# mjq11302010044/TPGSR

Hardware: AMD Instinct MI355X
Metric: training img/s (16x64->32x128, bs=48/GPU), TPGSR-TSRN full train step (higher is better)
Workload: dtype bf16x2; 1 GPU; C3: TPGSR-TSRN = TSRN_TL (STN+mask) + CRNN teacher/student text prior, stu_iter 1, full train step (teacher fwd, student fwd+bwd, distill loss, prior dropout, SR fwd+bwd, ImageLoss(gradient), clip 0.25, Adam); tpg=crnn, batch_per_gpu=48, global_batch=48, parallelism=dp1, launch=recorded plans, plain launches: main + weight-gradient + teacher streams

## Files before the change

### tpgsr_amd/csrc/gru_wgrad.hip

```cpp
#include "conv_xbf_common.h"
#include <mutex>
#include <stdlib.h>

#define GW_PITCH 832
#define GW_ROWS 32
#define GW_PLANE (GW_ROWS * GW_PITCH)
#define GW_HP 96
#define GW_GI 160
#define GW_GN 352

__device__ __forceinline__ bf16x8 gw_frag(const unsigned char* plane, int lane, int col0, int mb) {
  const int G = lane >> 4, q = lane & 15;
  const int mbase = mb * 16 + (G >> 1) * 8;
  const int c0 = col0 + (G & 1) * 16 + (q & 3) * 4;
  const unsigned char* p = plane + (mbase + (q >> 2)) * GW_PITCH + c0 * 2;
  s16x4 lo = __builtin_amdgcn_ds_read_tr16_b64_v4i16((lds_s16x4_ptr)(p));
  s16x4 hi = __builtin_amdgcn_ds_read_tr16_b64_v4i16((lds_s16x4_ptr)(p + 4 * GW_PITCH));
  typedef short s16x8 __attribute__((ext_vector_type(8)));
  s16x8 v = __builtin_shufflevector(lo, hi, 0, 1, 2, 3, 4, 5, 6, 7);
  return __builtin_bit_cast(bf16x8, v);
}

template <int LD, int T, int KB>
__global__ __launch_bounds__(384) void gru_wgrad_kernel(tpgsr_gru_wgrad_args w, int P, int MB) {
  extern __shared__ __attribute__((aligned(16))) unsigned char gsm[];
  const tpgsr_conv_args& a = w.c;
  const int tid = threadIdx.x;
  const int lane = tid & 63, wave = __builtin_amdgcn_readfirstlane(tid >> 6);
  const int z = blockIdx.x, Z = gridDim.x;
  const int mbeg = z * MB, mend = min(P, mbeg + MB);
  constexpr int QA = KB * 8;

  const bool doA = tid < 16 * QA;
  const int a_cq = doA ? tid % QA : 0, a_r0 = doA ? tid / QA : 0;
  const bool doH = tid < 256;
  const int h_cq = tid & 15, h_r0 = (tid >> 4) & 15;
  const bool doN = tid >= 128;
  const int n_cq = (tid - 128) & 15, n_r0 = ((tid - 128) >> 4) & 15;
  const int g_cq = tid % 48, g_r0 = tid / 48;

  const size_t in_floats = (size_t)a.N * a.H * a.W * a.in_ld;
  const __amdgpu_buffer_rsrc_t rs_in = make_rsrc(a.in, in_floats);
  const __amdgpu_buffer_rsrc_t rs_in2 = (LD & 16) ? make_rsrc(a.in_b, (size_t)a.N * a.W * a.in_b_ld)
                                                  : make_rsrc(a.in2 ? a.in2 : a.in, (size_t)a.N * a.H * a.W * a.in2_ld);
  const __amdgpu_buffer_rsrc_t rs_h = make_rsrc(w.h, (size_t)P * 64);
  const __amdgpu_buffer_rsrc_t rs_gi = make_rsrc(w.dgi, (size_t)P * 192);
  const __amdgpu_buffer_rsrc_t rs_gn = make_rsrc(w.dghn, (size_t)P * 64);
  float4 qs = make_float4(1.f, 1.f, 1.f, 1.f), qt = make_float4(0.f, 0.f, 0.f, 0.f);
  if ((LD & 1) && doA) {
    qs = *reinterpret_cast<const float4*>(a.in_scale + a_cq * 4);
    qt = *reinterpret_cast<const float4*>(a.in_shift + a_cq * 4);
  }
  const KPos kp = {0, 0, a_cq * 4};
  const int hd = h_cq >> 3;
  const int hstep = (w.axis == 0 ? 1 : a.W) * (hd == 0 ? -1 : 1);

  ARaw ra[2];
  float4 rh[2], rn[2], rg[4];
  float4 dbq = make_float4(0.f, 0.f, 0.f, 0.f), dbn = make_float4(0.f, 0.f, 0.f, 0.f);
  auto load_chunk = [&](const int mc) __attribute__((always_inline)) {
#pragma unroll
    for (int i = 0; i < 2; ++i) {
      if (doA) {
        const PixelPos p = decode_pixel(a, mc + a_r0 + 16 * i, mend);
        ra[i] = load_a_raw<LD>(a, rs_in, rs_in2, p, kp);
      }
      if (doH) {
        const int m = mc + h_r0 + 16 * i;
        const PixelPos p = decode_pixel(a, m, mend);
        const int pos = w.axis == 0 ? p.ow : p.oh, last = (w.axis == 0 ? a.W : a.H) - 1;
        const bool ok = p.valid && (hd == 0 ? pos > 0 : pos < last);
        rh[i] = buf_load4(rs_h, ok ? ((unsigned)(m + hstep) * 64u + (unsigned)(h_cq * 4)) * 4u : OOB_OFF);
      }
      if (doN) {
        const int m = mc + n_r0 + 16 * i;
        rn[i] = buf_load4(rs_gn, m < mend ? ((unsigned)m * 64u + (unsigned)(n_cq * 4)) * 4u : OOB_OFF);
      }
    }
#pragma unroll
    for (int i = 0; i < 4; ++i) {
      const int m = mc + g_r0 + 8 * i;
      rg[i] = buf_load4(rs_gi, m < mend ? ((unsigned)m * 192u + (unsigned)(g_cq * 4)) * 4u : OOB_OFF);
    }
  };
  auto put = [&](const float4& v, const int row, const int col) __attribute__((always_inline)) {
    uint2 hsp[T];
    split4<T>(v, hsp);
#pragma unroll
    for (int t = 0; t < T; ++t) *reinterpret_cast<uint2*>(gsm + t * GW_PLANE + row * GW_PITCH + col * 2) = hsp[t];
  };
  auto store_chunk = [&]() __attribute__((always_inline)) {
#pragma unroll
    for (int i = 0; i < 2; ++i) {
      if (doA) put(finish_a<LD>(a, ra[i], qs, qt), a_r0 + 16 * i, a_cq * 4);
      if (doH) put(rh[i], h_r0 + 16 * i, GW_HP + h_cq * 4);
      if (doN) {
        put(rn[i], n_r0 + 16 * i, GW_GN + n_cq * 4);
        dbn.x += rn[i].x; dbn.y += rn[i].y; dbn.z += rn[i].z; dbn.w += rn[i].w;
      }
    }
#pragma unroll
    for (int i = 0; i < 4; ++i) {
      put(rg[i], g_r0 + 8 * i, GW_GI + g_cq * 4);
      dbq.x += rg[i].x; dbq.y += rg[i].y; dbq.z += rg[i].z; dbq.w += rg[i].w;
    }
  };

  const int d = wave / 3, g = wave - 3 * d;
  floatx16 acc[KB], acch;
#pragma unroll
  for (int r = 0; r < 16; ++r) {
    acch[r] = 0.f;
#pragma unroll
    for (int kb = 0; kb < KB; ++kb) acc[kb][r] = 0.f;
  }

  if (mbeg < mend) {
    load_chunk(mbeg);
    store_chunk();
  }
  __syncthreads();
  for (int mc = mbeg; mc < mend; mc += GW_ROWS) {
    const bool more = mc + GW_ROWS < mend;
    if (more) load_chunk(mc + GW_ROWS);
#pragma unroll
    for (int mb = 0; mb < GW_ROWS / 16; ++mb) {
      bf16x8 by[T], byh[T], av[T];
#pragma unroll
      for (int t = 0; t < T; ++t) by[t] = gw_frag(gsm + t * GW_PLANE, lane, GW_GI + 32 * wave, mb);
      if (g == 2) {
#pragma unroll
        for (int t = 0; t < T; ++t) byh[t] = gw_frag(gsm + t * GW_PLANE, lane, GW_GN + 32 * d, mb);
      } else {
#pragma unroll
        for (int t = 0; t < T; ++t) byh[t] = by[t];
      }
#pragma unroll
      for (int kb = 0; kb < KB; ++kb) {
#pragma unroll
        for (int t = 0; t < T; ++t) av[t] = gw_frag(gsm + t * GW_PLANE, lane, 32 * kb, mb);
        acc[kb] = mfma_terms<T>(av, by, acc[kb]);
      }
#pragma unroll
      for (int t = 0; t < T; ++t) av[t] = gw_frag(gsm + t * GW_PLANE, lane, GW_HP + 32 * d, mb);
      acch = mfma_terms<T>(av, byh, acch);
    }
    __builtin_amdgcn_sched_barrier(0);
    __syncthreads();
    if (more) {
      store_chunk();
      __syncthreads();
    }
  }

  const int col = lane & 31;
#pragma unroll
  for (int kb = 0; kb < KB; ++kb) {
    float* dst = w.partC + ((size_t)z * a.Cin + 32 * kb) * 192 + 32 * wave + col;
#pragma unroll
    for (int r = 0; r < 16; ++r) dst[(size_t)((r & 3) + 8 * (r >> 2) + 4 * (lane >> 5)) * 192] = acc[kb][r];
  }
  {
    float* dst = w.partH + ((size_t)d * Z + z) * 32 * 96 + 32 * g + col;
#pragma unroll
    for (int r = 0; r < 16; ++r) dst[(size_t)((r & 3) + 8 * (r >> 2) + 4 * (lane >> 5)) * 96] = acch[r];
  }
  float* red = reinterpret_cast<float*>(gsm);
  float* redn = red + 8 * 192;
  *reinterpret_cast<float4*>(red + g_r0 * 192 + g_cq * 4) = dbq;
  if (doN) *reinterpret_cast<float4*>(redn + n_r0 * 64 + n_cq * 4) = dbn;
  __syncthreads();
  if (tid < 192) {
    float s = 0.f;
#pragma unroll
    for (int r = 0; r < 8; ++r) s += red[r * 192 + tid];
    w.dbC[(size_t)z * 192 + tid] = s;
    const int dd = tid / 96, c = tid - 96 * dd;
    if (c < 64) w.dbH[((size_t)dd * Z + z) * 96 + c] = s;
  } else if (tid < 256) {
    const int c = tid - 192;
    float s = 0.f;
#pragma unroll
    for (int r = 0; r < 16; ++r) s += redn[r * 64 + c];
    w.dbH[((size_t)(c >> 5) * Z + z) * 96 + 64 + (c & 31)] = s;
  }
}

static int g_gw_z = [] { const char* e = getenv("TPGSR_GRU_WGRAD_Z"); const int v = e ? atoi(e) : 128; return v > 0 ? v : 128; }();

extern "C" int tpgsr_gru_wgrad_splits(long long P) {
  long long z = g_gw_z;
  const long long maxz = (P + 63) / 64;
  if (z > maxz) z = maxz;
  if (z < 1) z = 1;
  const long long mb = ((P + z - 1) / z + GW_ROWS - 1) / GW_ROWS * GW_ROWS;
  return (int)((P + mb - 1) / mb);
}

extern "C" int tpgsr_gru_wgrad(const tpgsr_gru_wgrad_args* w, void* stream) {
  TPGSR_CHECK_ARG(w != nullptr, "tpgsr_gru_wgrad: null args");
  const tpgsr_conv_args* a = &w->c;
  TPGSR_CHECK_ARG(a->in && w->dgi && w->dghn && w->h && w->partC && w->partH && w->dbC && w->dbH, "tpgsr_gru_wgrad: null pointer");
  TPGSR_CHECK_ARG(a->N > 0 && a->H > 0 && a->W > 0 && (a->Cin == 64 || a->Cin == 96) && a->Cout == 192 && a->KH == 1 && a->KW == 1 &&
                      a->pad_h == 0 && a->pad_w == 0 && a->OH == a->H && a->OW == a->W && (w->axis == 0 || w->axis == 1),
                  "tpgsr_gru_wgrad: geometry (Cin %d must be 64 | 96, Cout %d must be 192, 1x1, axis %d)", a->Cin, a->Cout, w->axis);
  TPGSR_CHECK_ARG(a->terms >= 1 && a->terms <= 3, "tpgsr_gru_wgrad: runs on the split-bf16 matrix-core path only (terms %d)", a->terms);
  TPGSR_CHECK_ARG(!a->in_ps && !a->in_act && a->in_dil_w <= 1 && a->stride_w <= 1 && (a->in_ld & 3) == 0 && (a->in_coff & 3) == 0 &&
                      ((uintptr_t)a->in & 15) == 0, "tpgsr_gru_wgrad: unsupported loader (pixel shuffle / activation / dilation / unaligned rows)");
  TPGSR_CHECK_ARG((a->in_scale == nullptr) == (a->in_shift == nullptr), "tpgsr_gru_wgrad: in_scale / in_shift must come together");
  if (a->in_b)
    TPGSR_CHECK_ARG(a->cin_a > 0 && a->cin_a < a->Cin && (a->cin_a & 3) == 0 && a->in_b_ld >= a->Cin - a->cin_a && (a->in_b_ld & 3) == 0 && !a->in2,
                    "tpgsr_gru_wgrad: bad concat description");
  TPGSR_CHECK_ARG(a->in_ld >= (a->in_b ? a->cin_a : a->Cin) + a->in_coff, "tpgsr_gru_wgrad: in_ld too small");
  if (a->in2) TPGSR_CHECK_ARG(a->in2_ld >= a->Cin && (a->in2_ld & 3) == 0, "tpgsr_gru_wgrad: bad in2_ld");
  const long long P = (long long)a->N * a->H * a->W;
  TPGSR_CHECK_ARG(P * 192 * 4 <= 0x7fffffffll && P * a->in_ld * 4 <= 0x7fffffffll, "tpgsr_gru_wgrad: operand exceeds the 2 GiB buffer-addressing window (%lld pixels)", P);
  const int Z = w->zsplits;
  TPGSR_CHECK_ARG(Z > 0, "tpgsr_gru_wgrad: zsplits must be the caller's tpgsr_gru_wgrad_splits(P)");
  const int MB = (int)(((P + Z - 1) / Z + GW_ROWS - 1) / GW_ROWS * GW_ROWS);
  TPGSR_CHECK_ARG((long long)MB * Z >= P, "tpgsr_gru_wgrad: %d splits do not cover %lld pixels", Z, P);
  const int ld = (a->in_scale ? 1 : 0) | (a->in2 ? 4 : 0) | (a->in_b ? 16 : 0);
  const int T = a->terms, KB = a->Cin / 32;
  const void* fn = nullptr;
#define GW_PICK(L, K_)                                                                                        \
  fn = T == 1 ? (const void*)gru_wgrad_kernel<L, 1, K_> : T == 2 ? (const void*)gru_wgrad_kernel<L, 2, K_> \
                                                                   : (const void*)gru_wgrad_kernel<L, 3, K_>;
  if (ld == 0 && KB == 2) { GW_PICK(0, 2) }
  else if (ld == 1 && KB == 2) { GW_PICK(1, 2) }
  else if (ld == 4 && KB == 2) { GW_PICK(4, 2) }
  else if (ld == 17 && KB == 3) { GW_PICK(17, 3) }
  else if (ld == 0 && KB == 3) { GW_PICK(0, 3) }
#undef GW_PICK
  TPGSR_CHECK_ARG(fn != nullptr, "tpgsr_gru_wgrad: no kernel for loader %d with %d input channels", ld, a->Cin);
  const size_t lds = (size_t)T * GW_PLANE;
  if (lds > 64 * 1024) {
    static std::mutex mu;
    static const void* done[64][8];
    int dev = 0;
    if (hipGetDevice(&dev) != hipSuccess || dev < 0 || dev >= 64) {
      tpgsr_set_error("tpgsr_gru_wgrad: hipGetDevice failed");
      return TPGSR_ERR_LAUNCH;
    }
    std::lock_guard<std::mutex> lock(mu);
    bool seen = false;
    int free_slot = -1;
    for (int i = 0; i < 8; ++i) {
      if (done[dev][i] == fn) seen = true;
      if (!done[dev][i] && free_slot < 0) free_slot = i;
    }
    if (!seen) {
      if (hipFuncSetAttribute(fn, hipFuncAttributeMaxDynamicSharedMemorySize, (int)lds) != hipSuccess) {
        tpgsr_set_error("tpgsr_gru_wgrad: LDS opt-in (%zu bytes) failed", lds);
        return TPGSR_ERR_LAUNCH;
      }
      if (free_slot >= 0) done[dev][free_slot] = fn;
    }
  }
  tpgsr_gru_wgrad_args args = *w;
  int Pi = (int)P, MBi = MB;
  void* params[] = {&args, &Pi, &MBi};
  if (hipLaunchKernel(fn, dim3(Z), dim3(384), params, lds, (hipStream_t)stream) != hipSuccess) {
    tpgsr_set_error("tpgsr_gru_wgrad: launch failed: %s", hipGetErrorString(hipGetLastError()));
    return TPGSR_ERR_LAUNCH;
  }
  return 0;
}
```

Measured before the change: 8865 img/s.

## Double-buffer register prefetch in GRU weight-gradient kernel with branchless loads

Restructures the GRU wgrad main loop to keep two register stages and prefetch two chunks ahead, unrolling by two so global loads for chunk i+2 overlap the MFMA contraction of chunk i. Load guards become branchless through out-of-bounds offsets, and the hidden-gate fragment selection becomes a computed column instead of a divergent branch. Scheduling barriers are added per sub-block to constrain interleaving. The extra stage raises register pressure and may cut occupancy. The unrolled loop also processes an odd trailing chunk whose rows are all masked.

```diff
diff --git a/tpgsr_amd/csrc/gru_wgrad.hip b/tpgsr_amd/csrc/gru_wgrad.hip
--- a/tpgsr_amd/csrc/gru_wgrad.hip
+++ b/tpgsr_amd/csrc/gru_wgrad.hip
@@ -55,32 +55,35 @@
   const int hd = h_cq >> 3;
   const int hstep = (w.axis == 0 ? 1 : a.W) * (hd == 0 ? -1 : 1);
 
-  ARaw ra[2];
-  float4 rh[2], rn[2], rg[4];
+  struct Stage {
+    ARaw ra[2];
+    float4 rh[2], rn[2], rg[4];
+  };
+  Stage s0, s1;
   float4 dbq = make_float4(0.f, 0.f, 0.f, 0.f), dbn = make_float4(0.f, 0.f, 0.f, 0.f);
-  auto load_chunk = [&](const int mc) __attribute__((always_inline)) {
+  auto load_chunk = [&](Stage& s, const int mc) __attribute__((always_inline)) {
 #pragma unroll
     for (int i = 0; i < 2; ++i) {
-      if (doA) {
-        const PixelPos p = decode_pixel(a, mc + a_r0 + 16 * i, mend);
-        ra[i] = load_a_raw<LD>(a, rs_in, rs_in2, p, kp);
-      }
-      if (doH) {
+      {
+        const PixelPos p = decode_pixel(a, mc + a_r0 + 16 * i, doA ? mend : 0);
+        s.ra[i] = load_a_raw<LD>(a, rs_in, rs_in2, p, kp);
+      }
+      {
         const int m = mc + h_r0 + 16 * i;
-        const PixelPos p = decode_pixel(a, m, mend);
+        const PixelPos p = decode_pixel(a, m, doH ? mend : 0);
         const int pos = w.axis == 0 ? p.ow : p.oh, last = (w.axis == 0 ? a.W : a.H) - 1;
         const bool ok = p.valid && (hd == 0 ? pos > 0 : pos < last);
-        rh[i] = buf_load4(rs_h, ok ? ((unsigned)(m + hstep) * 64u + (unsigned)(h_cq * 4)) * 4u : OOB_OFF);
-      }
-      if (doN) {
+        s.rh[i] = buf_load4(rs_h, ok ? ((unsigned)(m + hstep) * 64u + (unsigned)(h_cq * 4)) * 4u : OOB_OFF);
+      }
+      {
         const int m = mc + n_r0 + 16 * i;
-        rn[i] = buf_load4(rs_gn, m < mend ? ((unsigned)m * 64u + (unsigned)(n_cq * 4)) * 4u : OOB_OFF);
+        s.rn[i] = buf_load4(rs_gn, doN && m < mend ? ((unsigned)m * 64u + (unsigned)(n_cq * 4)) * 4u : OOB_OFF);
       }
     }
 #pragma unroll
     for (int i = 0; i < 4; ++i) {
       const int m = mc + g_r0 + 8 * i;
-      rg[i] = buf_load4(rs_gi, m < mend ? ((unsigned)m * 192u + (unsigned)(g_cq * 4)) * 4u : OOB_OFF);
+      s.rg[i] = buf_load4(rs_gi, m < mend ? ((unsigned)m * 192u + (unsigned)(g_cq * 4)) * 4u : OOB_OFF);
     }
   };
   auto put = [&](const float4& v, const int row, const int col) __attribute__((always_inline)) {
@@ -89,20 +92,20 @@
 #pragma unroll
     for (int t = 0; t < T; ++t) *reinterpret_cast<uint2*>(gsm + t * GW_PLANE + row * GW_PITCH + col * 2) = hsp[t];
   };
-  auto store_chunk = [&]() __attribute__((always_inline)) {
+  auto store_chunk = [&](const Stage& s) __attribute__((always_inline)) {
 #pragma unroll
     for (int i = 0; i < 2; ++i) {
-      if (doA) put(finish_a<LD>(a, ra[i], qs, qt), a_r0 + 16 * i, a_cq * 4);
-      if (doH) put(rh[i], h_r0 + 16 * i, GW_HP + h_cq * 4);
+      if (doA) put(finish_a<LD>(a, s.ra[i], qs, qt), a_r0 + 16 * i, a_cq * 4);
+      if (doH) put(s.rh[i], h_r0 + 16 * i, GW_HP + h_cq * 4);
       if (doN) {
-        put(rn[i], n_r0 + 16 * i, GW_GN + n_cq * 4);
-        dbn.x += rn[i].x; dbn.y += rn[i].y; dbn.z += rn[i].z; dbn.w += rn[i].w;
+        put(s.rn[i], n_r0 + 16 * i, GW_GN + n_cq * 4);
+        dbn.x += s.rn[i].x; dbn.y += s.rn[i].y; dbn.z += s.rn[i].z; dbn.w += s.rn[i].w;
       }
     }
 #pragma unroll
     for (int i = 0; i < 4; ++i) {
-      put(rg[i], g_r0 + 8 * i, GW_GI + g_cq * 4);
-      dbq.x += rg[i].x; dbq.y += rg[i].y; dbq.z += rg[i].z; dbq.w += rg[i].w;
+      put(s.rg[i], g_r0 + 8 * i, GW_GI + g_cq * 4);
+      dbq.x += s.rg[i].x; dbq.y += s.rg[i].y; dbq.z += s.rg[i].z; dbq.w += s.rg[i].w;
     }
   };
 
@@ -115,42 +118,43 @@
     for (int kb = 0; kb < KB; ++kb) acc[kb][r] = 0.f;
   }
 
-  if (mbeg < mend) {
-    load_chunk(mbeg);
-    store_chunk();
-  }
-  __syncthreads();
-  for (int mc = mbeg; mc < mend; mc += GW_ROWS) {
-    const bool more = mc + GW_ROWS < mend;
-    if (more) load_chunk(mc + GW_ROWS);
+  const int hcol = g == 2 ? GW_GN + 32 * d : GW_GI + 32 * wave;
+  auto contract = [&]() __attribute__((always_inline)) {
 #pragma unroll
     for (int mb = 0; mb < GW_ROWS / 16; ++mb) {
       bf16x8 by[T], byh[T], av[T];
 #pragma unroll
       for (int t = 0; t < T; ++t) by[t] = gw_frag(gsm + t * GW_PLANE, lane, GW_GI + 32 * wave, mb);
-      if (g == 2) {
-#pragma unroll
-        for (int t = 0; t < T; ++t) byh[t] = gw_frag(gsm + t * GW_PLANE, lane, GW_GN + 32 * d, mb);
-      } else {
-#pragma unroll
-        for (int t = 0; t < T; ++t) byh[t] = by[t];
-      }
+#pragma unroll
+      for (int t = 0; t < T; ++t) byh[t] = gw_frag(gsm + t * GW_PLANE, lane, hcol, mb);
 #pragma unroll
       for (int kb = 0; kb < KB; ++kb) {
 #pragma unroll
         for (int t = 0; t < T; ++t) av[t] = gw_frag(gsm + t * GW_PLANE, lane, 32 * kb, mb);
         acc[kb] = mfma_terms<T>(av, by, acc[kb]);
+        if (T == 3 && KB == 3) __builtin_amdgcn_sched_barrier(0);
       }
 #pragma unroll
       for (int t = 0; t < T; ++t) av[t] = gw_frag(gsm + t * GW_PLANE, lane, GW_HP + 32 * d, mb);
       acch = mfma_terms<T>(av, byh, acch);
-    }
-    __builtin_amdgcn_sched_barrier(0);
+      __builtin_amdgcn_sched_barrier(0);
+    }
     __syncthreads();
-    if (more) {
-      store_chunk();
-      __syncthreads();
-    }
+  };
+
+  load_chunk(s0, mbeg);
+  load_chunk(s1, mbeg + GW_ROWS);
+  store_chunk(s0);
+  __syncthreads();
+  for (int mc = mbeg; mc < mend; mc += 2 * GW_ROWS) {
+    load_chunk(s0, mc + 2 * GW_ROWS);
+    contract();
+    store_chunk(s1);
+    __syncthreads();
+    load_chunk(s1, mc + 3 * GW_ROWS);
+    contract();
+    store_chunk(s0);
+    __syncthreads();
   }
 
   const int col = lane & 31;
```

Result: no change. 8784 img/s (-0.9%).
